# ZAX130/SmileCode

Measured on AMD Instinct MI355X. Metric: volume-pairs/sec (160x192x160) fwd+bwd, higher is better.
Workload: dtype f32; 1 GPU; ModeT 160x192x160 fp32, batch=1/GPU, full train step NCC+Grad3d fwd+bwd+Adam-amsgrad; global_batch=1, parallelism=dp1, allreduce=one flat all-reduce after backward

## Files before the change

smilecode_amd/csrc/warp.hip:

```cpp
#include "common.h"

namespace {

constexpr int BLK = 256;

template <int CPT> struct Vec;
template <> struct Vec<4> { using T = float4; };
template <> struct Vec<3> { using T = float3; };
template <> struct Vec<1> { using T = float; };

template <int CPT> __device__ __forceinline__ void ldv(const float* p, float (&r)[CPT]) {
  if constexpr (CPT == 4) {
    const float4 v = *reinterpret_cast<const float4*>(p);
    r[0] = v.x; r[1] = v.y; r[2] = v.z; r[3] = v.w;
  } else {
#pragma unroll
    for (int i = 0; i < CPT; ++i) r[i] = p[i];
  }
}
template <int CPT> __device__ __forceinline__ void stv(float* p, const float (&r)[CPT]) {
  if constexpr (CPT == 4) {
    *reinterpret_cast<float4*>(p) = make_float4(r[0], r[1], r[2], r[3]);
  } else {
#pragma unroll
// ... 436 lines not shown
          ICoff = off0 + sY;
        }
        if (want_flow) {
          if (add_flow && live) {
            gz += c == 0 ? go : 0.f; gy += c == 1 ? go : 0.f; gx += c == 2 ? go : 0.f;
          }
          for (int o = 1; o < G; o <<= 1) {
            gz += __shfl_xor(gz, o, 64);
            gy += __shfl_xor(gy, o, 64);
            gx += __shfl_xor(gx, o, 64);
          }
          const unsigned dfo = (inr && zin && yin && c == 0) ? (unsigned)n * 12u : WB_OOB;
          const wb_u32x3 ad = __builtin_amdgcn_raw_buffer_load_b96(r_da, dfo, 0, 0);
          const wb_u32x3 g3 = {__float_as_uint(gz + __uint_as_float(ad[0])), __float_as_uint(gy + __uint_as_float(ad[1])),
                               __float_as_uint(gx + __uint_as_float(ad[2]))};
          __builtin_amdgcn_raw_buffer_store_b96(g3, r_df, dfo, 0, 0);
        }
      }
      if (want_src) {
        atom(ICoff, IC[0][0]);
        if (__builtin_amdgcn_ballot_w64(IC[0][1] != 0.f)) atom(ICoff + sX, IC[0][1]);
        ON[YR][0] = IC[1][0]; ON[YR][1] = IC[1][1]; ONoff[YR] = ICoff == WB_NONE ? WB_NONE : ICoff + sZ;
#pragma unroll
        for (int k = 0; k <= YR; ++k) { OC[k][0] = ON[k][0]; OC[k][1] = ON[k][1]; OCoff[k] = ONoff[k]; }
      }
    }
    if (want_src) {
#pragma unroll
      for (int k = 0; k <= YR; ++k) { atom(OCoff[k], OC[k][0]); atom(OCoff[k] + sX, OC[k][1]); }
    }
  }
}

constexpr int G3Z = 4, G3Y = 4, G3X = 16, G3HZ = G3Z + 2, G3HY = G3Y + 2, G3HX = G3X + 2, G3HV = G3HZ * G3HY * G3HX;
__global__ __launch_bounds__(BLK) void warp_bwd_gather3_tiled_kernel(const float* __restrict__ src,
                                                                     const float* __restrict__ flow,
                                                                     const float* __restrict__ dout,
                                                                     float* __restrict__ dsrc, float* __restrict__ dflow,
                                                                     int D, int H, int W, int tiles_x, int tiles_y,
                                                                     int add_flow) {
  __shared__ __attribute__((aligned(8))) float fg[G3HV * 6];
  const int64_t V = (int64_t)D * H * W;
  const int b = blockIdx.y;
  int t = blockIdx.x;
  const int x0 = (t % tiles_x) * G3X; t /= tiles_x;
  const int y0 = (t % tiles_y) * G3Y;
  const int z0 = (t / tiles_y) * G3Z;
  constexpr int G3N = (G3HV * 3 + BLK - 1) / BLK;
  float2 stg[G3N];
#pragma unroll
  for (int j = 0; j < G3N; ++j) {
    const int i = min((int)threadIdx.x + j * BLK, G3HV * 3 - 1);
    const int v = i / 3, part = i - v * 3;
    const int hx = v % G3HX, r = v / G3HX;
    const int hy = r % G3HY, hz = r / G3HY;
    const int z = z0 + hz - 1, y = y0 + hy - 1, x = x0 + hx - 1;
    const bool in = z >= 0 && z < D && y >= 0 && y < H && x >= 0 && x < W;
    const int64_t n = (int64_t)b * V + (in ? ((int64_t)z * H + y) * W + x : 0);
    const float* pa = part == 0 ? flow + n * 3 : (part == 1 ? flow + n * 3 + 2 : dout + n * 3 + 1);
    const float* pb = part == 0 ? flow + n * 3 + 1 : (part == 1 ? dout + n * 3 : dout + n * 3 + 2);
    const float va = *pa, vb = *pb;
    stg[j] = in ? make_float2(va, vb) : make_float2(0.f, 0.f);
  }
#pragma unroll
  for (int j = 0; j < G3N; ++j) {
    const int i = threadIdx.x + j * BLK;
    if (i < G3HV * 3) *reinterpret_cast<float2*>(fg + i * 2) = stg[j];
  }
  __syncthreads();
  const int tx = threadIdx.x % G3X, ty = (threadIdx.x / G3X) % G3Y, tz = threadIdx.x / (G3X * G3Y);
  const int zi = z0 + tz, yi = y0 + ty, xi = x0 + tx;
  if (zi >= D || yi >= H || xi >= W) return;
  const int64_t n = (int64_t)b * V + ((int64_t)zi * H + yi) * W + xi;
  const int lc = ((tz + 1) * G3HY + ty + 1) * G3HX + tx + 1;
  if (dsrc) {
    float a0 = 0.f, a1 = 0.f, a2 = 0.f;
#pragma unroll
    for (int dz = -1; dz <= 1; ++dz)
#pragma unroll
      for (int dy = -1; dy <= 1; ++dy)
#pragma unroll
        for (int dx = -1; dx <= 1; ++dx) {
          const float* p = fg + (lc + (dz * G3HY + dy) * G3HX + dx) * 6;
          const float2 q0 = *reinterpret_cast<const float2*>(p), q1 = *reinterpret_cast<const float2*>(p + 2),
                       q2 = *reinterpret_cast<const float2*>(p + 4);
          const float wz = 1.f - fabsf((float)dz + q0.x);
          const float wy = 1.f - fabsf((float)dy + q0.y);
          const float wx = 1.f - fabsf((float)dx + q1.x);
          if (wz > 0.f && wy > 0.f && wx > 0.f) {
            const float wgt = wz * wy * wx;
            a0 = fmaf(wgt, q1.y, a0); a1 = fmaf(wgt, q2.x, a1); a2 = fmaf(wgt, q2.y, a2);
          }
        }
    float* dp = dsrc + n * 3;
    dp[0] = a0; dp[1] = a1; dp[2] = a2;
  }
  if (dflow) {
    const float* pc = fg + lc * 6;
    const Tri tr = tri_setup((float)zi + pc[0], (float)yi + pc[1], (float)xi + pc[2]);
    const float g0 = pc[3], g1 = pc[4], g2 = pc[5];
    const float* sb = src + (int64_t)b * V * 3;
    float gz = 0.f, gy = 0.f, gx = 0.f;
    float sp[8][3];
    bool okc[8];
#pragma unroll
    for (int q = 0; q < 8; ++q) {
      const int zz = tr.z0 + (q >> 2), yy = tr.y0 + ((q >> 1) & 1), xx = tr.x0 + (q & 1);
      okc[q] = zz >= 0 && zz < D && yy >= 0 && yy < H && xx >= 0 && xx < W;
      const float* pq = sb + (okc[q] ? (((int64_t)zz * H + yy) * W + xx) * 3 : 0);
      sp[q][0] = pq[0]; sp[q][1] = pq[1]; sp[q][2] = pq[2];
    }
#pragma unroll
    for (int dz = 0; dz < 2; ++dz) {
      const float wz = dz ? tr.fz : 1.f - tr.fz;
#pragma unroll
      for (int dy = 0; dy < 2; ++dy) {
        const float wy = dy ? tr.fy : 1.f - tr.fy;
#pragma unroll
        for (int dx = 0; dx < 2; ++dx) {
          const float wx = dx ? tr.fx : 1.f - tr.fx;
          const int q = dz * 4 + dy * 2 + dx;
          const float dot = okc[q] ? sp[q][0] * g0 + sp[q][1] * g1 + sp[q][2] * g2 : 0.f;
          gz += (dz ? 1.f : -1.f) * wy * wx * dot;
          gy += (dy ? 1.f : -1.f) * wz * wx * dot;
          gx += (dx ? 1.f : -1.f) * wz * wy * dot;
        }
      }
    }
    if (add_flow) { gz += g0; gy += g1; gx += g2; }
    float* dfp = dflow + n * 3;
    dfp[0] = gz; dfp[1] = gy; dfp[2] = gx;
  }
}

struct Lin { int i0, i1; float l0, l1; };
__device__ __forceinline__ Lin lin_src(int o, float ratio, int n_in) {
  Lin r;
  const float real = ratio * (float)o;
  r.i0 = min((int)real, n_in - 1);
  r.l1 = fminf(fmaxf(real - (float)r.i0, 0.f), 1.f);
  r.i1 = r.i0 + (r.i0 < n_in - 1 ? 1 : 0);
  r.l0 = 1.f - r.l1;
  return r;
}
__host__ __device__ __forceinline__ float up_ratio(int n_in) {
  return n_in > 1 ? (float)(n_in - 1) / (float)(2 * n_in - 1) : 0.f;
}

template <int CPT>
__global__ __launch_bounds__(BLK) void upsample2_fwd_kernel(const float* __restrict__ x, float* __restrict__ y, int d,
                                                            int h, int w, int C, int G, int64_t total, float scale) {
  const int D = 2 * d, H = 2 * h, W = 2 * w;
  const float rz = up_ratio(d), ry = up_ratio(h), rx = up_ratio(w);
  const int64_t Vo = (int64_t)D * H * W, Vi = (int64_t)d * h * w;
  const bool small = total < (1ll << 31) && Vo < (1ll << 31);
  for (int64_t idx = (int64_t)blockIdx.x * BLK + threadIdx.x; idx < total; idx += (int64_t)gridDim.x * BLK) {
    int g, xo, yo, zo;
    int64_t n, b;
    if (small) {
      const unsigned u = (unsigned)idx, un = u / (unsigned)G;
      g = (int)(u - un * (unsigned)G);
      const unsigned ub = un / (unsigned)Vo, uv = un - ub * (unsigned)Vo;
      const unsigned t2 = uv / (unsigned)W;
      xo = (int)(uv - t2 * (unsigned)W);
      zo = (int)(t2 / (unsigned)H);
      yo = (int)(t2 - (unsigned)zo * (unsigned)H);
      n = un; b = ub;
    } else {
      g = (int)(idx % G);
      n = idx / G;
      b = n / Vo;
      const int64_t v = n - b * Vo;
      xo = (int)(v % W);
      const int64_t t2 = v / W;
      yo = (int)(t2 % H); zo = (int)(t2 / H);
    }
    const Lin lz = lin_src(zo, rz, d), ly = lin_src(yo, ry, h), lx = lin_src(xo, rx, w);
    const float* xb = x + b * Vi * C + g * CPT;
    float acc[CPT];
#pragma unroll
    for (int c = 0; c < CPT; ++c) acc[c] = 0.f;
#pragma unroll
    for (int a = 0; a < 2; ++a)
#pragma unroll
      for (int bb = 0; bb < 2; ++bb)
#pragma unroll
        for (int cc = 0; cc < 2; ++cc) {
          const int zz = a ? lz.i1 : lz.i0, yy = bb ? ly.i1 : ly.i0, xx = cc ? lx.i1 : lx.i0;
          const float wgt = (a ? lz.l1 : lz.l0) * (bb ? ly.l1 : ly.l0) * (cc ? lx.l1 : lx.l0);
          float s[CPT];
          ldv<CPT>(xb + (((int64_t)zz * h + yy) * w + xx) * C, s);
#pragma unroll
          for (int c = 0; c < CPT; ++c) acc[c] = fmaf(wgt, s[c], acc[c]);
        }
#pragma unroll
    for (int c = 0; c < CPT; ++c) acc[c] *= scale;
    stv<CPT>(y + n * C + g * CPT, acc);
  }
}

__device__ __forceinline__ float lin_wt(int o, int i, float ratio, int n_in) {
  const Lin l = lin_src(o, ratio, n_in);
  return (l.i0 == i ? l.l0 : 0.f) + (l.i1 == i ? l.l1 : 0.f);
}
__device__ __forceinline__ void lin_range(int i, float ratio, int n_in, int& lo, int& hi) {
  const int n_out = 2 * n_in;
  if (ratio <= 0.f) { lo = 0; hi = n_out - 1; return; }
  lo = max(0, (int)floorf((float)(i - 1) / ratio) - 1);
  hi = min(n_out - 1, (int)ceilf((float)(i + 1) / ratio) + 1);
}

template <int CPT>
__global__ __launch_bounds__(BLK) void upsample2_bwd_kernel(const float* __restrict__ dy, float* __restrict__ dx, int d,
                                                            int h, int w, int C, int G, int64_t total, float scale) {
  const int H = 2 * h, W = 2 * w;
  const float rz = up_ratio(d), ry = up_ratio(h), rx = up_ratio(w);
  const int64_t Vo = (int64_t)8 * d * h * w, Vi = (int64_t)d * h * w;
  const int kx = threadIdx.x & 7;
  const int64_t stride = (int64_t)gridDim.x * (BLK / 8);
  for (int64_t idx = (int64_t)blockIdx.x * (BLK / 8) + (threadIdx.x >> 3); idx < total; idx += stride) {
    const int g = (int)(idx % G);
    const int64_t n = idx / G;
    const int64_t b = n / Vi, v = n - b * Vi;
    const int xi = (int)(v % w);
    const int64_t t2 = v / w;
    const int yi = (int)(t2 % h), zi = (int)(t2 / h);
    int zlo, zhi, ylo, yhi, xlo, xhi;
    lin_range(zi, rz, d, zlo, zhi);
    lin_range(yi, ry, h, ylo, yhi);
    lin_range(xi, rx, w, xlo, xhi);
    const float* gb = dy + b * Vo * C + g * CPT;
    float acc[CPT];
#pragma unroll
    for (int c = 0; c < CPT; ++c) acc[c] = 0.f;
    for (int xo = xlo + kx; xo <= xhi; xo += 8) {
      const float wx = lin_wt(xo, xi, rx, w);
      if (wx == 0.f) continue;
      for (int zo = zlo; zo <= zhi; ++zo) {
        const float wz = lin_wt(zo, zi, rz, d);
        if (wz == 0.f) continue;
        for (int yo = ylo; yo <= yhi; ++yo) {
          const float wy = lin_wt(yo, yi, ry, h);
          if (wy == 0.f) continue;
          float s[CPT];
          ldv<CPT>(gb + (((int64_t)zo * H + yo) * W + xo) * C, s);
          const float wgt = wz * wy * wx;
#pragma unroll
          for (int c = 0; c < CPT; ++c) acc[c] = fmaf(wgt, s[c], acc[c]);
        }
      }
    }
#pragma unroll
    for (int c = 0; c < CPT; ++c) {
      float r = acc[c];
      r += __shfl_xor(r, 1, 64); r += __shfl_xor(r, 2, 64); r += __shfl_xor(r, 4, 64);
      acc[c] = r * scale;
    }
    if (kx == 0) stv<CPT>(dx + n * C + g * CPT, acc);
  }
}

template <bool V4>
__global__ __launch_bounds__(BLK) void upsample2_bwd_rows_kernel(const float* __restrict__ in, float* __restrict__ out, int n,
                                                                 int64_t inner, float scale) {
  const float r = up_ratio(n);
  const int i = blockIdx.x % n;
  const int64_t o = blockIdx.x / n;
  int lo, hi;
  lin_range(i, r, n, lo, hi);
  while (lo < hi && lin_wt(lo, i, r, n) == 0.f) ++lo;
  float wt[9];
#pragma unroll
  for (int a = 0; a < 9; ++a) wt[a] = lo + a <= hi ? lin_wt(lo + a, i, r, n) : 0.f;
  const int cnt = hi - lo + 1;
  const float* p = in + (o * 2 * n + lo) * inner;
  float* q = out + (int64_t)blockIdx.x * inner;
  constexpr int E = V4 ? 4 : 1;
  for (int64_t k = ((int64_t)blockIdx.y * BLK + threadIdx.x) * E; k < inner; k += (int64_t)gridDim.y * BLK * E) {
    float acc[E];
#pragma unroll
    for (int e = 0; e < E; ++e) acc[e] = 0.f;
    float v4[4][E];
#pragma unroll
    for (int a = 0; a < 4; ++a) {
      const int aa = a < cnt ? a : cnt - 1;
      if (V4) {
        const float4 t = *reinterpret_cast<const float4*>(p + aa * inner + k);
        v4[a][0] = t.x; if (E > 1) { v4[a][1] = t.y; v4[a][2] = t.z; v4[a][3] = t.w; }
      } else {
        v4[a][0] = p[aa * inner + k];
      }
    }
#pragma unroll
    for (int a = 0; a < 4; ++a)
#pragma unroll
      for (int e = 0; e < E; ++e) acc[e] = fmaf(wt[a], v4[a][e], acc[e]);
#pragma unroll
    for (int a = 4; a < 9; ++a) {
      if (wt[a] == 0.f) continue;
      float v[E];
      if (V4) {
        const float4 t = *reinterpret_cast<const float4*>(p + a * inner + k);
        v[0] = t.x; if (E > 1) { v[1] = t.y; v[2] = t.z; v[3] = t.w; }
      } else {
        v[0] = p[a * inner + k];
      }
#pragma unroll
      for (int e = 0; e < E; ++e) acc[e] = fmaf(wt[a], v[e], acc[e]);
    }
    if (V4) *reinterpret_cast<float4*>(q + k) = make_float4(acc[0] * scale, acc[E > 1 ? 1 : 0] * scale, acc[E > 1 ? 2 : 0] * scale,
                                                            acc[E > 1 ? 3 : 0] * scale);
    else q[k] = acc[0] * scale;
  }
}

__global__ __launch_bounds__(BLK) void upsample2_bwd_axis_kernel(const float* __restrict__ in, float* __restrict__ out, int n,
                                                                 int inner, int64_t total, float scale) {
  const float r = up_ratio(n);
  for (int64_t idx = (int64_t)blockIdx.x * BLK + threadIdx.x; idx < total; idx += (int64_t)gridDim.x * BLK) {
    const int64_t t = idx / inner;
    const int k = (int)(idx - t * inner);
    const int i = (int)(t % n);
    const int64_t o = t / n;
    int lo, hi;
    lin_range(i, r, n, lo, hi);
    const float* p = in + (o * 2 * n) * inner + k;
    float acc = 0.f;
    for (int f = lo; f <= hi; ++f) {
      const float wgt = lin_wt(f, i, r, n);
      if (wgt != 0.f) acc = fmaf(wgt, p[(int64_t)f * inner], acc);
    }
    out[idx] = acc * scale;
  }
}

__global__ __launch_bounds__(BLK) void ncdhw_to_cl_kernel(const float* __restrict__ x, float* __restrict__ y, int C,
                                                          int64_t V, int64_t total) {
  for (int64_t idx = (int64_t)blockIdx.x * BLK + threadIdx.x; idx < total; idx += (int64_t)gridDim.x * BLK) {
    const int64_t b = idx / V, v = idx - b * V;
    for (int c = 0; c < C; ++c) y[idx * C + c] = x[(b * C + c) * V + v];
  }
}
__global__ __launch_bounds__(BLK) void cl_to_ncdhw_kernel(const float* __restrict__ x, float* __restrict__ y, int C,
                                                          int64_t V, int64_t total) {
  for (int64_t idx = (int64_t)blockIdx.x * BLK + threadIdx.x; idx < total; idx += (int64_t)gridDim.x * BLK) {
    const int64_t b = idx / V, v = idx - b * V;
    for (int c = 0; c < C; ++c) y[(b * C + c) * V + v] = x[idx * C + c];
  }
}

template <int HEADS>
__global__ __launch_bounds__(BLK) void cwm_tail_fwd_kernel(const float* __restrict__ x, const float* __restrict__ lg,
                                                           float* __restrict__ out, int64_t N) {
  for (int64_t n = (int64_t)blockIdx.x * BLK + threadIdx.x; n < N; n += (int64_t)gridDim.x * BLK) {
    float l[HEADS];
    float m = -INFINITY;
#pragma unroll
    for (int i = 0; i < HEADS; ++i) { l[i] = lg[n * HEADS + i]; m = fmaxf(m, l[i]); }
    float s = 0.f;
#pragma unroll
    for (int i = 0; i < HEADS; ++i) { l[i] = __expf(l[i] - m); s += l[i]; }
    const float inv = 2.f / s;
    float o0 = 0.f, o1 = 0.f, o2 = 0.f;
#pragma unroll
    for (int i = 0; i < HEADS; ++i) {
// ... 91 lines not shown
  DISPATCH_CPT(cpt, warp_fwd_kernel, flat_grid(total, BLK), (hipStream_t)stream, src, flow, out, D, H, W, C, G, total,
               mode, add_flow);
  return modet_launch_status();
}

#ifdef MODET_TUNING
int modet_debug_warp_census(unsigned long long* buf) {
  return (int)hipMemcpyToSymbol(HIP_SYMBOL(g_wb_dbg), &buf, sizeof(buf));
}
#endif

int modet_warp_bwd(const float* src, const float* flow, const float* d_out, float* d_src, float* d_flow, int B, int D,
                   int H, int W, int C, int add_flow, int flow_bound, modet_stream_t stream) {
  return modet_warp_bwd_t(src, 0, flow, d_out, d_src, d_flow, B, D, H, W, C, add_flow, flow_bound, stream);
}

int modet_warp_bwd_t(const void* srcv, int src_bf16, const float* flow, const float* d_out, float* d_src, float* d_flow, int B,
                     int D, int H, int W, int C, int add_flow, int flow_bound, modet_stream_t stream) {
  return modet_warp_bwd_acc(srcv, src_bf16, flow, d_out, d_src, d_flow, nullptr, B, D, H, W, C, add_flow, flow_bound, stream);
}

int modet_warp_bwd_acc(const void* srcv, int src_bf16, const float* flow, const float* d_out, float* d_src, float* d_flow,
                       const float* d_flow_add, int B, int D, int H, int W, int C, int add_flow, int flow_bound,
                       modet_stream_t stream) {
  const float* src = (const float*)srcv;
  if (d_flow_add && (!d_flow || flow_bound != 0)) return MODET_ERR_UNSUPPORTED;
  MODET_CHECK_PTR(src); MODET_CHECK_PTR(flow); MODET_CHECK_PTR(d_out);
  MODET_CHECK_DIM(B > 0 && D > 0 && H > 0 && W > 0 && C > 0);
  if (add_flow && C != 3) return MODET_ERR_DIM;
  if (flow_bound != 0 && (flow_bound != 1 || C != 3)) return MODET_ERR_UNSUPPORTED;
  if (src_bf16 && (add_flow || flow_bound)) return MODET_ERR_UNSUPPORTED;
  if (!d_src && !d_flow) return MODET_OK;
  if (flow_bound == 1) {
    const int tx = cdiv(W, G3X), ty = cdiv(H, G3Y), tz = cdiv(D, G3Z);
    hipLaunchKernelGGL(warp_bwd_gather3_tiled_kernel, dim3(tx * ty * tz, B), dim3(BLK), 0, (hipStream_t)stream, src, flow,
                       d_out, d_src, d_flow, D, H, W, tx, ty, add_flow);
    return modet_launch_status();
  }
  int G = 1;
  while (G < C) G <<= 1;
  if (G > 64) return MODET_ERR_UNSUPPORTED;
  hipStream_t s = (hipStream_t)stream;
  if (d_src) modet_zero_async(d_src, (size_t)B * D * H * W * C * sizeof(float), s);
  const int64_t total2 = (int64_t)B * cdiv(D, WB2_ZR) * cdiv(H, WB2_YR) * W * G;
  const char wb2 = modet_tuning_env("MODET_WARP_BWD2");
  if (d_src && wb2 != '0' && (int64_t)B * D * H * W * (C > 3 ? C : 3) * 4 < 0x7fffffffLL && (int64_t)(D + 3) * (H + 3) * (W + 3) < (1 << 23) &&
      W * C * 4 < (1 << 23) && total2 < 0x7fffffffLL && total2 >= 256 * 256) {
    if (src_bf16) hipLaunchKernelGGL((warp_bwd2_kernel<WB2_ZR, WB2_YR, true>), dim3(flat_grid(total2, BLK)), dim3(BLK), 0, s, src, flow,
                                     d_out, d_src, d_flow, d_flow_add, B, D, H, W, C, G, (unsigned)total2, add_flow);
    else hipLaunchKernelGGL((warp_bwd2_kernel<WB2_ZR, WB2_YR, false>), dim3(flat_grid(total2, BLK)), dim3(BLK), 0, s, src, flow, d_out,
                            d_src, d_flow, d_flow_add, B, D, H, W, C, G, (unsigned)total2, add_flow);
    return modet_launch_status();
  }
  const int64_t total = (int64_t)B * cdiv(D, ZRUN) * H * W * G;
  if (src_bf16) hipLaunchKernelGGL(warp_bwd_kernel<true>, dim3(flat_grid(total, BLK)), dim3(BLK), 0, s, src, flow, d_out, d_src, d_flow,
                                   d_flow_add, D, H, W, C, G, total, add_flow);
  else hipLaunchKernelGGL(warp_bwd_kernel<false>, dim3(flat_grid(total, BLK)), dim3(BLK), 0, s, src, flow, d_out, d_src, d_flow,
                          d_flow_add, D, H, W, C, G, total, add_flow);
  return modet_launch_status();
}

size_t modet_warp_bwd_det_ws_bytes(int B, int D, int H, int W, int C) {
  return 64 + (size_t)B * D * H * W * C * sizeof(long long);
}

int modet_warp_bwd_det(const void* srcv, int src_bf16, const float* flow, const float* d_out, float* d_src, float* d_flow,
                       const float* d_flow_add, void* ws, size_t ws_bytes, int B, int D, int H, int W, int C, int add_flow,
                       modet_stream_t stream) {
  const float* src = (const float*)srcv;
// ... 47 lines not shown
  else if (src_bf16) hipLaunchKernelGGL((warp_fwd_kernel<4, false, true>), grid, dim3(BLK), 0, s, sf, flow, of, D, H, W, C, G, total, 0, 0);
  else hipLaunchKernelGGL((warp_fwd_kernel<4, true, false>), grid, dim3(BLK), 0, s, sf, flow, of, D, H, W, C, G, total, 0, 0);
  return modet_launch_status();
}

int modet_warp_fwd_o16(const float* src, const float* flow, void* out_bf16, int B, int D, int H, int W, int C,
                       modet_stream_t stream) {
  return modet_warp_fwd_t(src, 0, flow, out_bf16, 1, B, D, H, W, C, stream);
}

int modet_upsample2_fwd(const float* x, float* y, int B, int d, int h, int w, int C, float scale,
                        modet_stream_t stream) {
  MODET_CHECK_PTR(x); MODET_CHECK_PTR(y);
  MODET_CHECK_DIM(B > 0 && d > 0 && h > 0 && w > 0 && C > 0);
  const int cpt = pick_cpt(C), G = C / cpt;
  const int64_t total = (int64_t)B * 8 * d * h * w * G;
  DISPATCH_CPT(cpt, upsample2_fwd_kernel, flat_grid(total, BLK), (hipStream_t)stream, x, y, d, h, w, C, G, total,
               scale);
  return modet_launch_status();
}

int modet_upsample2_bwd(const float* d_y, float* d_x, int B, int d, int h, int w, int C, float scale,
                        modet_stream_t stream) {
  MODET_CHECK_PTR(d_y); MODET_CHECK_PTR(d_x);
  MODET_CHECK_DIM(B > 0 && d > 0 && h > 0 && w > 0 && C > 0);
  const int cpt = pick_cpt(C), G = C / cpt;
  const int64_t total = (int64_t)B * d * h * w * G;
  DISPATCH_CPT(cpt, upsample2_bwd_kernel, flat_grid(total * 8, BLK), (hipStream_t)stream, d_y, d_x, d, h, w, C, G, total,
               scale);
  return modet_launch_status();
}

size_t modet_upsample2_bwd_sep_ws_bytes(int B, int d, int h, int w, int C) {
  if ((int64_t)B * d * h * w < 65536) return 0;
  return ((size_t)B * d * 2 * h * 2 * w * C + (size_t)B * d * h * 2 * w * C) * sizeof(float);
}

int modet_upsample2_bwd_sep(const float* d_y, float* d_x, void* ws, size_t ws_bytes, int B, int d, int h, int w, int C,
                            float scale, modet_stream_t stream) {
  MODET_CHECK_PTR(d_y); MODET_CHECK_PTR(d_x); MODET_CHECK_PTR(ws);
  MODET_CHECK_DIM(B > 0 && d > 0 && h > 0 && w > 0 && C > 0);
  const size_t need = modet_upsample2_bwd_sep_ws_bytes(B, d, h, w, C);
  if (need == 0) return MODET_ERR_UNSUPPORTED;
  if (ws_bytes < need) return MODET_ERR_WORKSPACE;
  hipStream_t s = (hipStream_t)stream;
  float* t1 = (float*)ws;
  float* t2 = t1 + (size_t)B * d * 2 * h * 2 * w * C;
  const int64_t in_z = (int64_t)4 * h * w * C, in_y = (int64_t)2 * w * C;
  const int64_t n1 = (int64_t)B * d * in_z, n2 = (int64_t)B * d * h * in_y, n3 = (int64_t)B * d * h * w * C;
  (void)n1; (void)n2;
  auto rows = [&](const float* in, float* out, int n, int64_t nrows, int64_t inner) {
    int gy = (int)cdiv64(inner, (int64_t)BLK * 4);
    if (gy > 64) gy = 64;
    if (inner % 4 == 0)
      hipLaunchKernelGGL(upsample2_bwd_rows_kernel<true>, dim3((unsigned)nrows, gy), dim3(BLK), 0, s, in, out, n, inner, 1.f);
    else
      hipLaunchKernelGGL(upsample2_bwd_rows_kernel<false>, dim3((unsigned)nrows, gy), dim3(BLK), 0, s, in, out, n, inner, 1.f);
  };
  rows(d_y, t1, d, (int64_t)B * d, in_z);
  rows(t1, t2, h, (int64_t)B * d * h, in_y);
  hipLaunchKernelGGL(upsample2_bwd_axis_kernel, dim3(flat_grid(n3, BLK)), dim3(BLK), 0, s, (const float*)t2, d_x, w, C, n3, scale);
  return modet_launch_status();
}

int modet_ncdhw_to_cl(const float* x, float* y, int B, int C, int64_t V, modet_stream_t stream) {
  MODET_CHECK_PTR(x); MODET_CHECK_PTR(y);
  MODET_CHECK_DIM(B > 0 && C > 0 && V > 0);
  const int64_t total = (int64_t)B * V;
  hipLaunchKernelGGL(ncdhw_to_cl_kernel, dim3(flat_grid(total, BLK)), dim3(BLK), 0, (hipStream_t)stream, x, y, C, V,
                     total);
  return modet_launch_status();
}

int modet_cl_to_ncdhw(const float* x, float* y, int B, int C, int64_t V, modet_stream_t stream) {
  MODET_CHECK_PTR(x); MODET_CHECK_PTR(y);
  MODET_CHECK_DIM(B > 0 && C > 0 && V > 0);
  const int64_t total = (int64_t)B * V;
  hipLaunchKernelGGL(cl_to_ncdhw_kernel, dim3(flat_grid(total, BLK)), dim3(BLK), 0, (hipStream_t)stream, x, y, C, V,
                     total);
  return modet_launch_status();
}

#define DISPATCH_HEADS(KERNEL, ...)                                                                               \
  switch (heads) {                                                                                                \
    case 1: hipLaunchKernelGGL(KERNEL<1>, dim3(flat_grid(N, BLK)), dim3(BLK), 0, (hipStream_t)stream, __VA_ARGS__); break; \
    case 2: hipLaunchKernelGGL(KERNEL<2>, dim3(flat_grid(N, BLK)), dim3(BLK), 0, (hipStream_t)stream, __VA_ARGS__); break; \
    case 4: hipLaunchKernelGGL(KERNEL<4>, dim3(flat_grid(N, BLK)), dim3(BLK), 0, (hipStream_t)stream, __VA_ARGS__); break; \
    case 8: hipLaunchKernelGGL(KERNEL<8>, dim3(flat_grid(N, BLK)), dim3(BLK), 0, (hipStream_t)stream, __VA_ARGS__); break; \
    default: return MODET_ERR_UNSUPPORTED;                                                                        \
  }

int modet_cwm_tail_fwd(const float* x, const float* logits, float* out, int64_t N, int heads, modet_stream_t stream) {
  MODET_CHECK_PTR(x); MODET_CHECK_PTR(logits); MODET_CHECK_PTR(out);
  MODET_CHECK_DIM(N > 0 && heads > 0);
// ... 29 lines not shown
```

Baseline: 141.7 volume-pairs/sec.

## Stream z-slices through LDS ring in warp bwd and fuse upsample bwd passes

The warp backward gather kernel now walks a z-column per block, keeping a 4-slot shared-memory ring of flow/dout/src planes and prefetching the next plane with buffer loads while the current one is computed. This removes the 3x halo re-reads in z of the old 4x4x16 tiles and serves most src corner lookups from LDS. Separately, the three-pass separable upsample backward, which went through global workspaces, is replaced by one tiled kernel that does the z, y and x reductions in shared memory. A buffer-load fast path is also added to upsample forward for 3-channel inputs. Costs are more shared memory per block, fewer blocks in flight, and a per-slice barrier.

After: 141.8 volume-pairs/sec (median of 6 runs). No clear change (+0.1%).

```diff
diff --git a/smilecode_amd/csrc/warp.hip b/smilecode_amd/csrc/warp.hip
--- a/smilecode_amd/csrc/warp.hip
+++ b/smilecode_amd/csrc/warp.hip
@@ -492,104 +492,154 @@
   }
 }
 
-constexpr int G3Z = 4, G3Y = 4, G3X = 16, G3HZ = G3Z + 2, G3HY = G3Y + 2, G3HX = G3X + 2, G3HV = G3HZ * G3HY * G3HX;
+constexpr int G3Y = 8, G3X = 32, G3HY = G3Y + 2, G3HX = G3X + 2, G3HV = G3HY * G3HX, G3RING = 4;
+constexpr int G3NL = (G3HV + BLK - 1) / BLK;
+static_assert(G3Y * G3X == BLK, "one thread per voxel of the tile");
 __global__ __launch_bounds__(BLK) void warp_bwd_gather3_tiled_kernel(const float* __restrict__ src,
                                                                      const float* __restrict__ flow,
                                                                      const float* __restrict__ dout,
                                                                      float* __restrict__ dsrc, float* __restrict__ dflow,
-                                                                     int D, int H, int W, int tiles_x, int tiles_y,
+                                                                     int D, int H, int W, int tiles_x, int tiles_y, int zc,
                                                                      int add_flow) {
-  __shared__ __attribute__((aligned(8))) float fg[G3HV * 6];
-  const int64_t V = (int64_t)D * H * W;
+  __shared__ __attribute__((aligned(16))) float fg[G3RING][G3HV * 6];
+  __shared__ __attribute__((aligned(16))) float sr[G3RING][G3HV * 3];
+  const int HW = H * W;
+  const int64_t V3 = (int64_t)D * HW * 3;
   const int b = blockIdx.y;
   int t = blockIdx.x;
   const int x0 = (t % tiles_x) * G3X; t /= tiles_x;
   const int y0 = (t % tiles_y) * G3Y;
-  const int z0 = (t / tiles_y) * G3Z;
-  constexpr int G3N = (G3HV * 3 + BLK - 1) / BLK;
-  float2 stg[G3N];
-#pragma unroll
-  for (int j = 0; j < G3N; ++j) {
-    const int i = min((int)threadIdx.x + j * BLK, G3HV * 3 - 1);
-    const int v = i / 3, part = i - v * 3;
-    const int hx = v % G3HX, r = v / G3HX;
-    const int hy = r % G3HY, hz = r / G3HY;
-    const int z = z0 + hz - 1, y = y0 + hy - 1, x = x0 + hx - 1;
-    const bool in = z >= 0 && z < D && y >= 0 && y < H && x >= 0 && x < W;
-    const int64_t n = (int64_t)b * V + (in ? ((int64_t)z * H + y) * W + x : 0);
-    const float* pa = part == 0 ? flow + n * 3 : (part == 1 ? flow + n * 3 + 2 : dout + n * 3 + 1);
-    const float* pb = part == 0 ? flow + n * 3 + 1 : (part == 1 ? dout + n * 3 : dout + n * 3 + 2);
-    const float va = *pa, vb = *pb;
-    stg[j] = in ? make_float2(va, vb) : make_float2(0.f, 0.f);
-  }
-#pragma unroll
-  for (int j = 0; j < G3N; ++j) {
-    const int i = threadIdx.x + j * BLK;
-    if (i < G3HV * 3) *reinterpret_cast<float2*>(fg + i * 2) = stg[j];
+  const int zs = (t / tiles_y) * zc, ze = min(zs + zc, D);
+  const unsigned vbytes = (unsigned)V3 * 4u;
+  const bool want_src = dsrc != nullptr, want_flow = dflow != nullptr;
+  const WbRsrc r_src = wb_rsrc(src + b * V3, vbytes), r_flow = wb_rsrc(flow + b * V3, vbytes), r_do = wb_rsrc(dout + b * V3, vbytes);
+  const WbRsrc r_ds = wb_rsrc(want_src ? dsrc + b * V3 : nullptr, want_src ? vbytes : 0u);
+  const WbRsrc r_df = wb_rsrc(want_flow ? dflow + b * V3 : nullptr, want_flow ? vbytes : 0u);
+  unsigned soff[G3NL];
+#pragma unroll
+  for (int r = 0; r < G3NL; ++r) {
+    const int v = (int)threadIdx.x + r * BLK;
+    const int hy = v / G3HX, hx = v - hy * G3HX;
+    const int y = y0 + hy - 1, x = x0 + hx - 1;
+    soff[r] = (v < G3HV && y >= 0 && y < H && x >= 0 && x < W) ? (unsigned)(y * W + x) * 12u : WB_OOB;
+  }
+  struct Stage { wb_u32x3 f[G3NL], g[G3NL], s[G3NL]; };
+  auto issue = [&](int p, Stage& st) {
+    const bool zok = p >= 0 && p < D;
+    const unsigned pb = zok ? (unsigned)p * (unsigned)HW * 12u : 0u;
+#pragma unroll
+    for (int r = 0; r < G3NL; ++r) {
+      const unsigned off = (zok && soff[r] != WB_OOB) ? pb + soff[r] : WB_OOB;
+      st.f[r] = __builtin_amdgcn_raw_buffer_load_b96(r_flow, off, 0, 0);
+      st.g[r] = __builtin_amdgcn_raw_buffer_load_b96(r_do, off, 0, 0);
+      if (want_flow) st.s[r] = __builtin_amdgcn_raw_buffer_load_b96(r_src, off, 0, 0);
+    }
+  };
+  auto commit = [&](int p, const Stage& st) {
+    float* fq = fg[(p + 1) & (G3RING - 1)];
+    float* sq = sr[(p + 1) & (G3RING - 1)];
+#pragma unroll
+    for (int r = 0; r < G3NL; ++r) {
+      const int v = (int)threadIdx.x + r * BLK;
+      if (v < G3HV) {
+        *reinterpret_cast<float2*>(fq + v * 6) = make_float2(__uint_as_float(st.f[r][0]), __uint_as_float(st.f[r][1]));
+        *reinterpret_cast<float2*>(fq + v * 6 + 2) = make_float2(__uint_as_float(st.f[r][2]), __uint_as_float(st.g[r][0]));
+        *reinterpret_cast<float2*>(fq + v * 6 + 4) = make_float2(__uint_as_float(st.g[r][1]), __uint_as_float(st.g[r][2]));
+        if (want_flow) {
+          sq[v * 3] = __uint_as_float(st.s[r][0]); sq[v * 3 + 1] = __uint_as_float(st.s[r][1]); sq[v * 3 + 2] = __uint_as_float(st.s[r][2]);
+        }
+      }
+    }
+  };
+  {
+    Stage a, c, e;
+    issue(zs - 1, a); issue(zs, c); issue(zs + 1, e);
+    commit(zs - 1, a); commit(zs, c); commit(zs + 1, e);
   }
   __syncthreads();
-  const int tx = threadIdx.x % G3X, ty = (threadIdx.x / G3X) % G3Y, tz = threadIdx.x / (G3X * G3Y);
-  const int zi = z0 + tz, yi = y0 + ty, xi = x0 + tx;
-  if (zi >= D || yi >= H || xi >= W) return;
-  const int64_t n = (int64_t)b * V + ((int64_t)zi * H + yi) * W + xi;
-  const int lc = ((tz + 1) * G3HY + ty + 1) * G3HX + tx + 1;
-  if (dsrc) {
-    float a0 = 0.f, a1 = 0.f, a2 = 0.f;
-#pragma unroll
-    for (int dz = -1; dz <= 1; ++dz)
-#pragma unroll
-      for (int dy = -1; dy <= 1; ++dy)
-#pragma unroll
-        for (int dx = -1; dx <= 1; ++dx) {
-          const float* p = fg + (lc + (dz * G3HY + dy) * G3HX + dx) * 6;
-          const float2 q0 = *reinterpret_cast<const float2*>(p), q1 = *reinterpret_cast<const float2*>(p + 2),
-                       q2 = *reinterpret_cast<const float2*>(p + 4);
-          const float wz = 1.f - fabsf((float)dz + q0.x);
-          const float wy = 1.f - fabsf((float)dy + q0.y);
-          const float wx = 1.f - fabsf((float)dx + q1.x);
-          if (wz > 0.f && wy > 0.f && wx > 0.f) {
-            const float wgt = wz * wy * wx;
-            a0 = fmaf(wgt, q1.y, a0); a1 = fmaf(wgt, q2.x, a1); a2 = fmaf(wgt, q2.y, a2);
+  const int tx = threadIdx.x % G3X, ty = threadIdx.x / G3X;
+  const int yi = y0 + ty, xi = x0 + tx;
+  const bool active = yi < H && xi < W;
+  const int lc = (ty + 1) * G3HX + tx + 1;
+  const unsigned nrow = active ? (unsigned)(yi * W + xi) * 12u : WB_OOB;
+  for (int zi = zs; zi < ze; ++zi) {
+    Stage nx;
+    const bool more = zi + 2 <= ze;
+    if (more) issue(zi + 2, nx);
+    const float* fz[3] = {fg[zi & (G3RING - 1)], fg[(zi + 1) & (G3RING - 1)], fg[(zi + 2) & (G3RING - 1)]};
+    const unsigned n = active ? (unsigned)zi * (unsigned)HW * 12u + nrow : WB_OOB;
+    if (want_src) {
+      float a0 = 0.f, a1 = 0.f, a2 = 0.f;
+#pragma unroll
+      for (int dz = -1; dz <= 1; ++dz)
+#pragma unroll
+        for (int dy = -1; dy <= 1; ++dy)
+#pragma unroll
+          for (int dx = -1; dx <= 1; ++dx) {
+            const float* p = fz[dz + 1] + (lc + dy * G3HX + dx) * 6;
+            const float2 q0 = *reinterpret_cast<const float2*>(p), q1 = *reinterpret_cast<const float2*>(p + 2),
+                         q2 = *reinterpret_cast<const float2*>(p + 4);
+            const float wz = 1.f - fabsf((float)dz + q0.x);
+            const float wy = 1.f - fabsf((float)dy + q0.y);
+            const float wx = 1.f - fabsf((float)dx + q1.x);
+            if (wz > 0.f && wy > 0.f && wx > 0.f) {
+              const float wgt = wz * wy * wx;
+              a0 = fmaf(wgt, q1.y, a0); a1 = fmaf(wgt, q2.x, a1); a2 = fmaf(wgt, q2.y, a2);
+            }
           }
-        }
-    float* dp = dsrc + n * 3;
-    dp[0] = a0; dp[1] = a1; dp[2] = a2;
-  }
-  if (dflow) {
-    const float* pc = fg + lc * 6;
-    const Tri tr = tri_setup((float)zi + pc[0], (float)yi + pc[1], (float)xi + pc[2]);
-    const float g0 = pc[3], g1 = pc[4], g2 = pc[5];
-    const float* sb = src + (int64_t)b * V * 3;
-    float gz = 0.f, gy = 0.f, gx = 0.f;
-    float sp[8][3];
-    bool okc[8];
-#pragma unroll
-    for (int q = 0; q < 8; ++q) {
-      const int zz = tr.z0 + (q >> 2), yy = tr.y0 + ((q >> 1) & 1), xx = tr.x0 + (q & 1);
-      okc[q] = zz >= 0 && zz < D && yy >= 0 && yy < H && xx >= 0 && xx < W;
-      const float* pq = sb + (okc[q] ? (((int64_t)zz * H + yy) * W + xx) * 3 : 0);
-      sp[q][0] = pq[0]; sp[q][1] = pq[1]; sp[q][2] = pq[2];
-    }
-#pragma unroll
-    for (int dz = 0; dz < 2; ++dz) {
-      const float wz = dz ? tr.fz : 1.f - tr.fz;
-#pragma unroll
-      for (int dy = 0; dy < 2; ++dy) {
-        const float wy = dy ? tr.fy : 1.f - tr.fy;
-#pragma unroll
-        for (int dx = 0; dx < 2; ++dx) {
-          const float wx = dx ? tr.fx : 1.f - tr.fx;
-          const int q = dz * 4 + dy * 2 + dx;
-          const float dot = okc[q] ? sp[q][0] * g0 + sp[q][1] * g1 + sp[q][2] * g2 : 0.f;
-          gz += (dz ? 1.f : -1.f) * wy * wx * dot;
-          gy += (dy ? 1.f : -1.f) * wz * wx * dot;
-          gx += (dx ? 1.f : -1.f) * wz * wy * dot;
-        }
-      }
-    }
-    if (add_flow) { gz += g0; gy += g1; gx += g2; }
-    float* dfp = dflow + n * 3;
-    dfp[0] = gz; dfp[1] = gy; dfp[2] = gx;
+      const wb_u32x3 o3 = {__float_as_uint(a0), __float_as_uint(a1), __float_as_uint(a2)};
+      __builtin_amdgcn_raw_buffer_store_b96(o3, r_ds, n, 0, 0);
+    }
+    if (want_flow) {
+      const float* pc = fz[1] + lc * 6;
+      const Tri tr = tri_setup((float)zi + pc[0], (float)yi + pc[1], (float)xi + pc[2]);
+      const float g0 = pc[3], g1 = pc[4], g2 = pc[5];
+      float gz = 0.f, gy = 0.f, gx = 0.f;
+      float sp[8][3];
+      bool okc[8];
+#pragma unroll
+      for (int q = 0; q < 8; ++q) {
+        const int zz = tr.z0 + (q >> 2), yy = tr.y0 + ((q >> 1) & 1), xx = tr.x0 + (q & 1);
+        okc[q] = zz >= 0 && zz < D && yy >= 0 && yy < H && xx >= 0 && xx < W;
+      }
+      const int wz0 = tr.z0 - (zi - 1), wy0 = tr.y0 - (y0 - 1), wx0 = tr.x0 - (x0 - 1);
+      if (wz0 >= 0 && wz0 <= 1 && wy0 >= 0 && wy0 <= G3HY - 2 && wx0 >= 0 && wx0 <= G3HX - 2) {
+#pragma unroll
+        for (int q = 0; q < 8; ++q) {
+          const float* pq = sr[(tr.z0 + (q >> 2) + 1) & (G3RING - 1)] + ((wy0 + ((q >> 1) & 1)) * G3HX + wx0 + (q & 1)) * 3;
+          sp[q][0] = pq[0]; sp[q][1] = pq[1]; sp[q][2] = pq[2];
+        }
+      } else {
+#pragma unroll
+        for (int q = 0; q < 8; ++q) {
+          const int zz = tr.z0 + (q >> 2), yy = tr.y0 + ((q >> 1) & 1), xx = tr.x0 + (q & 1);
+          const wb_u32x3 s3 = __builtin_amdgcn_raw_buffer_load_b96(r_src, okc[q] ? (unsigned)((zz * H + yy) * W + xx) * 12u : WB_OOB, 0, 0);
+          sp[q][0] = __uint_as_float(s3[0]); sp[q][1] = __uint_as_float(s3[1]); sp[q][2] = __uint_as_float(s3[2]);
+        }
+      }
+#pragma unroll
+      for (int dz = 0; dz < 2; ++dz) {
+        const float wz = dz ? tr.fz : 1.f - tr.fz;
+#pragma unroll
+        for (int dy = 0; dy < 2; ++dy) {
+          const float wy = dy ? tr.fy : 1.f - tr.fy;
+#pragma unroll
+          for (int dx = 0; dx < 2; ++dx) {
+            const float wx = dx ? tr.fx : 1.f - tr.fx;
+            const int q = dz * 4 + dy * 2 + dx;
+            const float dot = okc[q] ? sp[q][0] * g0 + sp[q][1] * g1 + sp[q][2] * g2 : 0.f;
+            gz += (dz ? 1.f : -1.f) * wy * wx * dot;
+            gy += (dy ? 1.f : -1.f) * wz * wx * dot;
+            gx += (dx ? 1.f : -1.f) * wz * wy * dot;
+          }
+        }
+      }
+      if (add_flow) { gz += g0; gy += g1; gx += g2; }
+      const wb_u32x3 o3 = {__float_as_uint(gz), __float_as_uint(gy), __float_as_uint(gx)};
+      __builtin_amdgcn_raw_buffer_store_b96(o3, r_df, n, 0, 0);
+    }
+    if (more) commit(zi + 2, nx);
+    __syncthreads();
   }
 }
 
@@ -614,6 +664,34 @@
   const float rz = up_ratio(d), ry = up_ratio(h), rx = up_ratio(w);
   const int64_t Vo = (int64_t)D * H * W, Vi = (int64_t)d * h * w;
   const bool small = total < (1ll << 31) && Vo < (1ll << 31);
+  if constexpr (CPT == 3) {
+    if (G == 1 && total * 12 < (1ll << 31)) {
+      const WbRsrc r_x = wb_rsrc(x, (unsigned)(total / 8 * 12)), r_y = wb_rsrc(y, (unsigned)(total * 12));
+      for (unsigned u = blockIdx.x * BLK + threadIdx.x; u < (unsigned)total; u += gridDim.x * BLK) {
+        const unsigned ub = u / (unsigned)Vo, uv = u - ub * (unsigned)Vo;
+        const unsigned t2 = uv / (unsigned)W;
+        const int xo = (int)(uv - t2 * (unsigned)W), zo = (int)(t2 / (unsigned)H), yo = (int)(t2 - (unsigned)zo * (unsigned)H);
+        const Lin lz = lin_src(zo, rz, d), ly = lin_src(yo, ry, h), lx = lin_src(xo, rx, w);
+        const unsigned xb = ub * (unsigned)Vi;
+        wb_u32x3 s[8];
+#pragma unroll
+        for (int q = 0; q < 8; ++q) {
+          const int zz = (q >> 2) ? lz.i1 : lz.i0, yy = ((q >> 1) & 1) ? ly.i1 : ly.i0, xx = (q & 1) ? lx.i1 : lx.i0;
+          s[q] = __builtin_amdgcn_raw_buffer_load_b96(r_x, (xb + (unsigned)((zz * h + yy) * w + xx)) * 12u, 0, 0);
+        }
+        float acc[3] = {0.f, 0.f, 0.f};
+#pragma unroll
+        for (int q = 0; q < 8; ++q) {
+          const float wgt = ((q >> 2) ? lz.l1 : lz.l0) * (((q >> 1) & 1) ? ly.l1 : ly.l0) * ((q & 1) ? lx.l1 : lx.l0);
+#pragma unroll
+          for (int c = 0; c < 3; ++c) acc[c] = fmaf(wgt, __uint_as_float(s[q][c]), acc[c]);
+        }
+        const wb_u32x3 o3 = {__float_as_uint(acc[0] * scale), __float_as_uint(acc[1] * scale), __float_as_uint(acc[2] * scale)};
+        __builtin_amdgcn_raw_buffer_store_b96(o3, r_y, u * 12u, 0, 0);
+      }
+      return;
+    }
+  }
   for (int64_t idx = (int64_t)blockIdx.x * BLK + threadIdx.x; idx < total; idx += (int64_t)gridDim.x * BLK) {
     int g, xo, yo, zo;
     int64_t n, b;
@@ -663,11 +741,12 @@
   const Lin l = lin_src(o, ratio, n_in);
   return (l.i0 == i ? l.l0 : 0.f) + (l.i1 == i ? l.l1 : 0.f);
 }
-__device__ __forceinline__ void lin_range(int i, float ratio, int n_in, int& lo, int& hi) {
+__host__ __device__ __forceinline__ void lin_range(int i, float ratio, int n_in, int& lo, int& hi) {
   const int n_out = 2 * n_in;
   if (ratio <= 0.f) { lo = 0; hi = n_out - 1; return; }
-  lo = max(0, (int)floorf((float)(i - 1) / ratio) - 1);
-  hi = min(n_out - 1, (int)ceilf((float)(i + 1) / ratio) + 1);
+  const int a = (int)floorf((float)(i - 1) / ratio) - 1, b = (int)ceilf((float)(i + 1) / ratio) + 1;
+  lo = a > 0 ? a : 0;
+  hi = b < n_out - 1 ? b : n_out - 1;
 }
 
 template <int CPT>
@@ -720,77 +799,124 @@
   }
 }
 
-template <bool V4>
-__global__ __launch_bounds__(BLK) void upsample2_bwd_rows_kernel(const float* __restrict__ in, float* __restrict__ out, int n,
-                                                                 int64_t inner, float scale) {
+constexpr int UB_TY = 8, UB_TX = 16, UB_FY = 24, UB_FX = 40, UB_CC = 8, UB_ZC = 16, UB_TN = 16;
+static_assert(UB_TY <= UB_TN && UB_TX <= UB_TN && UB_ZC <= UB_TN, "one table row per index of a tile axis");
+inline bool up_tile_fits(int n, int T, int cap) {
   const float r = up_ratio(n);
-  const int i = blockIdx.x % n;
-  const int64_t o = blockIdx.x / n;
-  int lo, hi;
-  lin_range(i, r, n, lo, hi);
-  while (lo < hi && lin_wt(lo, i, r, n) == 0.f) ++lo;
-  float wt[9];
-#pragma unroll
-  for (int a = 0; a < 9; ++a) wt[a] = lo + a <= hi ? lin_wt(lo + a, i, r, n) : 0.f;
-  const int cnt = hi - lo + 1;
-  const float* p = in + (o * 2 * n + lo) * inner;
-  float* q = out + (int64_t)blockIdx.x * inner;
-  constexpr int E = V4 ? 4 : 1;
-  for (int64_t k = ((int64_t)blockIdx.y * BLK + threadIdx.x) * E; k < inner; k += (int64_t)gridDim.y * BLK * E) {
-    float acc[E];
-#pragma unroll
-    for (int e = 0; e < E; ++e) acc[e] = 0.f;
-    float v4[4][E];
-#pragma unroll
-    for (int a = 0; a < 4; ++a) {
-      const int aa = a < cnt ? a : cnt - 1;
-      if (V4) {
-        const float4 t = *reinterpret_cast<const float4*>(p + aa * inner + k);
-        v4[a][0] = t.x; if (E > 1) { v4[a][1] = t.y; v4[a][2] = t.z; v4[a][3] = t.w; }
-      } else {
-        v4[a][0] = p[aa * inner + k];
-      }
-    }
-#pragma unroll
-    for (int a = 0; a < 4; ++a)
-#pragma unroll
-      for (int e = 0; e < E; ++e) acc[e] = fmaf(wt[a], v4[a][e], acc[e]);
-#pragma unroll
-    for (int a = 4; a < 9; ++a) {
-      if (wt[a] == 0.f) continue;
-      float v[E];
-      if (V4) {
-        const float4 t = *reinterpret_cast<const float4*>(p + a * inner + k);
-        v[0] = t.x; if (E > 1) { v[1] = t.y; v[2] = t.z; v[3] = t.w; }
-      } else {
-        v[0] = p[a * inner + k];
-      }
-#pragma unroll
-      for (int e = 0; e < E; ++e) acc[e] = fmaf(wt[a], v[e], acc[e]);
-    }
-    if (V4) *reinterpret_cast<float4*>(q + k) = make_float4(acc[0] * scale, acc[E > 1 ? 1 : 0] * scale, acc[E > 1 ? 2 : 0] * scale,
-                                                            acc[E > 1 ? 3 : 0] * scale);
-    else q[k] = acc[0] * scale;
-  }
-}
-
-__global__ __launch_bounds__(BLK) void upsample2_bwd_axis_kernel(const float* __restrict__ in, float* __restrict__ out, int n,
-                                                                 int inner, int64_t total, float scale) {
-  const float r = up_ratio(n);
-  for (int64_t idx = (int64_t)blockIdx.x * BLK + threadIdx.x; idx < total; idx += (int64_t)gridDim.x * BLK) {
-    const int64_t t = idx / inner;
-    const int k = (int)(idx - t * inner);
-    const int i = (int)(t % n);
-    const int64_t o = t / n;
-    int lo, hi;
-    lin_range(i, r, n, lo, hi);
-    const float* p = in + (o * 2 * n) * inner + k;
-    float acc = 0.f;
-    for (int f = lo; f <= hi; ++f) {
-      const float wgt = lin_wt(f, i, r, n);
-      if (wgt != 0.f) acc = fmaf(wgt, p[(int64_t)f * inner], acc);
-    }
-    out[idx] = acc * scale;
+  for (int i0 = 0; i0 < n; i0 += T) {
+    const int i1 = (i0 + T < n ? i0 + T : n) - 1;
+    int lo, hi, lo1, hi1;
+    lin_range(i0, r, n, lo, hi);
+    lin_range(i1, r, n, lo1, hi1);
+    if (hi1 - lo + 1 > cap) return false;
+  }
+  return true;
+}
+__global__ __launch_bounds__(BLK) void upsample2_bwd_rows_kernel(const float* __restrict__ dy, float* __restrict__ dx, int d, int h,
+                                                                 int w, int C, int ty, int tx, int zc, int tiles_x, int tiles_y,
+                                                                 float scale) {
+  __shared__ float t1[UB_FY * UB_FX * UB_CC];
+  __shared__ float t2[UB_TY * UB_FX * UB_CC];
+  __shared__ int ti[3][UB_TN][3];
+  __shared__ float tw[3][UB_TN][9];
+  const int H2 = 2 * h, W2 = 2 * w;
+  const int tid = threadIdx.x, lane = tid & 63, wave = tid >> 6;
+  const int b = blockIdx.y;
+  const int c0 = blockIdx.z * UB_CC, cw = min(UB_CC, C - c0);
+  int t = blockIdx.x;
+  const int xi0 = (t % tiles_x) * tx; t /= tiles_x;
+  const int yi0 = (t % tiles_y) * ty;
+  const int zi0 = (t / tiles_y) * zc;
+  const int nz = min(zc, d - zi0), nty = min(ty, h - yi0), ntx = min(tx, w - xi0);
+  {
+    const int ax = tid >> 6, j = tid & 63;
+    const int cntj = ax == 0 ? nz : (ax == 1 ? nty : ntx);
+    if (ax < 3 && j < cntj) {
+      const int n = ax == 0 ? d : (ax == 1 ? h : w), i = (ax == 0 ? zi0 : (ax == 1 ? yi0 : xi0)) + j;
+      const float r = up_ratio(n);
+      int lo, hi;
+      lin_range(i, r, n, lo, hi);
+      while (lo < hi && lin_wt(lo, i, r, n) == 0.f) ++lo;
+      const int cnt = hi - lo + 1;
+      int top = cnt - 1 < 3 ? cnt - 1 : 3;
+#pragma unroll
+      for (int a = 0; a < 9; ++a) {
+        const float wt = lo + a <= hi ? lin_wt(lo + a, i, r, n) : 0.f;
+        tw[ax][j][a] = wt;
+        if (a >= 4 && wt != 0.f) top = a;
+      }
+      ti[ax][j][0] = lo; ti[ax][j][1] = cnt; ti[ax][j][2] = top;
+    }
+  }
+  __syncthreads();
+  int fylo = ti[1][0][0], fyhi = 0, fxlo = ti[2][0][0], fxhi = 0;
+  for (int j = 0; j < nty; ++j) { fylo = min(fylo, ti[1][j][0]); fyhi = max(fyhi, ti[1][j][0] + ti[1][j][2]); }
+  for (int j = 0; j < ntx; ++j) { fxlo = min(fxlo, ti[2][j][0]); fxhi = max(fxhi, ti[2][j][0] + ti[2][j][2]); }
+  const int nfy = fyhi - fylo + 1, nfx = fxhi - fxlo + 1;
+  const int rowlen = nfx * cw;
+  const bool contig = cw == C;
+  const int64_t Vi = (int64_t)d * h * w, Vo = 8 * Vi;
+  const float* gb = dy + (int64_t)b * Vo * C + (int64_t)fxlo * C + c0;
+  float* ob = dx + (int64_t)b * Vi * C + c0;
+  const int nout = nty * ntx * cw, ntc = ntx * cw;
+  for (int zl = 0; zl < nz; ++zl) {
+    {
+      const int lo = ti[0][zl][0], cnt = ti[0][zl][1];
+      float wt[9];
+#pragma unroll
+      for (int a = 0; a < 9; ++a) wt[a] = tw[0][zl][a];
+      for (int Y = wave; Y < nfy; Y += BLK / 64) {
+        const float* p = gb + ((int64_t)lo * H2 + fylo + Y) * W2 * C;
+        const int64_t zs = (int64_t)H2 * W2 * C;
+        for (int k = lane; k < rowlen; k += 64) {
+          const int ko = contig ? k : (k / cw) * C + k % cw;
+          float v4[4];
+#pragma unroll
+          for (int a = 0; a < 4; ++a) v4[a] = p[(a < cnt ? a : cnt - 1) * zs + ko];
+          float acc = 0.f;
+#pragma unroll
+          for (int a = 0; a < 4; ++a) acc = fmaf(wt[a], v4[a], acc);
+#pragma unroll
+          for (int a = 4; a < 9; ++a) {
+            if (wt[a] == 0.f) continue;
+            acc = fmaf(wt[a], p[a * zs + ko], acc);
+          }
+          t1[Y * rowlen + k] = acc;
+        }
+      }
+    }
+    __syncthreads();
+    for (int yl = wave; yl < nty; yl += BLK / 64) {
+      const int lo = ti[1][yl][0] - fylo, cnt = ti[1][yl][1];
+      float wt[9];
+#pragma unroll
+      for (int a = 0; a < 9; ++a) wt[a] = tw[1][yl][a];
+      for (int k = lane; k < rowlen; k += 64) {
+        const float* p = t1 + lo * rowlen + k;
+        float acc = 0.f;
+#pragma unroll
+        for (int a = 0; a < 4; ++a) acc = fmaf(wt[a], p[(a < cnt ? a : cnt - 1) * rowlen], acc);
+#pragma unroll
+        for (int a = 4; a < 9; ++a) {
+          if (wt[a] == 0.f) continue;
+          acc = fmaf(wt[a], p[a * rowlen], acc);
+        }
+        t2[yl * rowlen + k] = acc;
+      }
+    }
+    __syncthreads();
+    for (int e = tid; e < nout; e += BLK) {
+      const int yl = e / ntc, rem = e - yl * ntc;
+      const int xl = rem / cw, c = rem - xl * cw;
+      const float* p = t2 + yl * rowlen + (ti[2][xl][0] - fxlo) * cw + c;
+      float acc = 0.f;
+#pragma unroll
+      for (int a = 0; a < 9; ++a) {
+        const float wgt = tw[2][xl][a];
+        if (wgt != 0.f) acc = fmaf(wgt, p[a * cw], acc);
+      }
+      ob[((((int64_t)(zi0 + zl)) * h + yi0 + yl) * w + xi0 + xl) * C + c] = acc * scale;
+    }
   }
 }
 
@@ -948,9 +1074,14 @@
   if (src_bf16 && (add_flow || flow_bound)) return MODET_ERR_UNSUPPORTED;
   if (!d_src && !d_flow) return MODET_OK;
   if (flow_bound == 1) {
-    const int tx = cdiv(W, G3X), ty = cdiv(H, G3Y), tz = cdiv(D, G3Z);
-    hipLaunchKernelGGL(warp_bwd_gather3_tiled_kernel, dim3(tx * ty * tz, B), dim3(BLK), 0, (hipStream_t)stream, src, flow,
-                       d_out, d_src, d_flow, D, H, W, tx, ty, add_flow);
+    if ((int64_t)D * H * W * 12 >= 0x7fffffffLL || B > 65535) return MODET_ERR_UNSUPPORTED;
+    const int tx = cdiv(W, G3X), ty = cdiv(H, G3Y);
+    int zc = 16;
+    while (zc > 4 && (int64_t)tx * ty * B * cdiv(D, zc) < 1024) zc >>= 1;
+    const char zt = modet_tuning_env("MODET_G3_ZC");
+    if (zt >= '0' && zt <= '4') zc = 4 << (zt - '0');
+    hipLaunchKernelGGL(warp_bwd_gather3_tiled_kernel, dim3(tx * ty * cdiv(D, zc), B), dim3(BLK), 0, (hipStream_t)stream, src, flow,
+                       d_out, d_src, d_flow, D, H, W, tx, ty, zc, add_flow);
     return modet_launch_status();
   }
   int G = 1;
@@ -1064,8 +1195,9 @@
 }
 
 size_t modet_upsample2_bwd_sep_ws_bytes(int B, int d, int h, int w, int C) {
+  (void)C;
   if ((int64_t)B * d * h * w < 65536) return 0;
-  return ((size_t)B * d * 2 * h * 2 * w * C + (size_t)B * d * h * 2 * w * C) * sizeof(float);
+  return 256;
 }
 
 int modet_upsample2_bwd_sep(const float* d_y, float* d_x, void* ws, size_t ws_bytes, int B, int d, int h, int w, int C,
@@ -1075,23 +1207,17 @@
   const size_t need = modet_upsample2_bwd_sep_ws_bytes(B, d, h, w, C);
   if (need == 0) return MODET_ERR_UNSUPPORTED;
   if (ws_bytes < need) return MODET_ERR_WORKSPACE;
-  hipStream_t s = (hipStream_t)stream;
-  float* t1 = (float*)ws;
-  float* t2 = t1 + (size_t)B * d * 2 * h * 2 * w * C;
-  const int64_t in_z = (int64_t)4 * h * w * C, in_y = (int64_t)2 * w * C;
-  const int64_t n1 = (int64_t)B * d * in_z, n2 = (int64_t)B * d * h * in_y, n3 = (int64_t)B * d * h * w * C;
-  (void)n1; (void)n2;
-  auto rows = [&](const float* in, float* out, int n, int64_t nrows, int64_t inner) {
-    int gy = (int)cdiv64(inner, (int64_t)BLK * 4);
-    if (gy > 64) gy = 64;
-    if (inner % 4 == 0)
-      hipLaunchKernelGGL(upsample2_bwd_rows_kernel<true>, dim3((unsigned)nrows, gy), dim3(BLK), 0, s, in, out, n, inner, 1.f);
-    else
-      hipLaunchKernelGGL(upsample2_bwd_rows_kernel<false>, dim3((unsigned)nrows, gy), dim3(BLK), 0, s, in, out, n, inner, 1.f);
-  };
-  rows(d_y, t1, d, (int64_t)B * d, in_z);
-  rows(t1, t2, h, (int64_t)B * d * h, in_y);
-  hipLaunchKernelGGL(upsample2_bwd_axis_kernel, dim3(flat_grid(n3, BLK)), dim3(BLK), 0, s, (const float*)t2, d_x, w, C, n3, scale);
+  int ty = UB_TY, tx = UB_TX;
+  while (ty > 1 && !up_tile_fits(h, ty, UB_FY)) --ty;
+  while (tx > 1 && !up_tile_fits(w, tx, UB_FX)) --tx;
+  const int cch = cdiv(C, UB_CC);
+  if (!up_tile_fits(h, ty, UB_FY) || !up_tile_fits(w, tx, UB_FX) || B > 65535 || cch > 65535) return MODET_ERR_UNSUPPORTED;
+  const int tiles_x = cdiv(w, tx), tiles_y = cdiv(h, ty);
+  int zc = UB_ZC;
+  while (zc > 1 && (int64_t)tiles_x * tiles_y * B * cch * cdiv(d, zc) < 1024) zc >>= 1;
+  if ((int64_t)tiles_x * tiles_y * cdiv(d, zc) > 0x7fffffffLL) return MODET_ERR_UNSUPPORTED;
+  hipLaunchKernelGGL(upsample2_bwd_rows_kernel, dim3((unsigned)(tiles_x * tiles_y * cdiv(d, zc)), B, cch), dim3(BLK), 0,
+                     (hipStream_t)stream, d_y, d_x, d, h, w, C, ty, tx, zc, tiles_x, tiles_y, scale);
   return modet_launch_status();
 }
 
```
